# SamsungSAILMontreal/ghn3

Measured on AMD Instinct MI355X. Metric: predicted-params/sec (GHN fwd+bwd), ghn3xlm16, 256-node graphs, higher is better.
Workload: dtype f16; 1 GPU; ghn3xlm16 fwd+bwd, 1 synthetic 256-node graph(s) per GPU (seed 256000+), 86515016 predicted params per GPU, loss = sum of Frobenius norms of the predicted tensors; ghn_params=654365312, decoder_rows=1421, workspace_bytes=2436048640, zero_fill_bytes=2797339192, parallelism=dp1, index_mode=reference, loss=fused into the tile kernels

## Files before the change

### ghn3_amd/build.py

```python
import os
import subprocess
import sys
from concurrent.futures import ThreadPoolExecutor

HERE = os.path.dirname(os.path.abspath(__file__))
ROOT = os.path.dirname(HERE)
CSRC = os.path.join(HERE, 'csrc')
OUT_DIR = os.path.join(HERE, 'lib')
LIB = os.path.join(OUT_DIR, 'libghn3_hip.so')
SOURCES = ['gemm.hip', 'gemm_p8.hip', 'gemm_small.hip', 'gemm_x3.hip', 'gemm_x3d.hip', 'gemm_wg.hip', 'attention.hip', 'elementwise.hip', 'target_ops.hip', 'tnet_msa.hip', 'tnet_attn.hip', 'tnet_head.hip', 'tnet_wgrad.hip', 'tnet_join.hip', 'tnet_patch.hip', 'runtime.hip']
FLAGS = ['--offload-arch=gfx950', '-O3', '-std=c++17', '-fPIC', '-I' + os.path.join(ROOT, 'include'),
         '-I' + CSRC, '-Wno-unused-result'] + os.environ.get('GHN3_HIPCC_EXTRA', '').split()


def _hipcc():
    for cand in (os.environ.get('HIPCC'), '/opt/rocm/bin/hipcc', 'hipcc'):
        if cand and (os.path.isabs(cand) and os.path.exists(cand) or not os.path.isabs(cand)):
            return cand
    raise RuntimeError('hipcc not found')


def _stale(target, deps):
    if not os.path.exists(target):
        return True
    t = os.path.getmtime(target)
    return any(os.path.getmtime(d) > t for d in deps)


def source_hash():
    import hashlib
    h = hashlib.sha256()
    files = [os.path.join(CSRC, f) for f in sorted(os.listdir(CSRC)) if f.endswith(('.hip', '.h'))]
    files += [os.path.join(ROOT, 'include', 'ghn3_hip.h'), os.path.join(HERE, 'program.py')]
    for f in files:
        with open(f, 'rb') as fh:
            h.update(os.path.basename(f).encode() + b'\0' + fh.read())
    return h.hexdigest()[:16]


def build(force=False, verbose=True):
    os.makedirs(OUT_DIR, exist_ok=True)
    hipcc = _hipcc()
    headers = [os.path.join(ROOT, 'include', 'ghn3_hip.h'), os.path.join(CSRC, 'ghn3_internal.h'),
# ... 27 lines not shown
```

### ghn3_amd/csrc/ghn3_internal.h

```cpp
#pragma once
#include <hip/hip_runtime.h>
#include <stdint.h>
#include "ghn3_hip.h"

struct GemmProbDev {
    const float* A; const float* B; float* C;
    const float* bias; const float* residual; const float* aux_in; float* aux_out;
    const int* a_gather; const int* b_gather; const int* c_gather;
    int M, N, K, lda, ldb, ldc;
    int a_q, a_s, b_q, b_s, c_q, c_s;
    int bias_q, bias_s, bias_stride;
    int act, dact, flags;
    float alpha;
    int tile_start;
    int tiles_m, tiles_n;
    int ksplit, k_chunk;
    int order;
    int kq, ks;
    const int* lim;
    int lim_kind;
    int xcd_cols;
    int pin;
    int pin_first, pin_count;
    int pin_end, pin_total;
    const float* alpha_amax;
    int ln_kind;
    float ln_eps;
    const float* ln_p[6];
    const void* B2;
    const int* mtab;
};


int ghn3_gemm_init();
int ghn3_gemm_launch(const GemmProbDev* d_probs, int n_probs, int total_tiles, int a_mode, int b_mode,
                     int tile, int ctype, hipStream_t stream);

int ghn3_gemm_h16d_launch(const GemmProbDev* d_probs, int n_probs, int total_tiles, int tile, int ctype, int grid_cap,
                          hipStream_t stream);
int ghn3_gemm_p8_init();
int ghn3_gemm_p8_launch(const GemmProbDev* d_probs, int n_probs, int total_tiles, int ctype, int grid_cap,
                        hipStream_t stream);
int ghn3_gemm_p8w_launch(const GemmProbDev* d_probs, int n_probs, int total_tiles, int ctype, int grid_cap,
                         hipStream_t stream);
int ghn3_gemm_p8d_launch(const GemmProbDev* d_probs, int n_probs, int total_tiles, int ctype, int grid_cap,
                         hipStream_t stream);
int ghn3_gemm_x3_init();
int ghn3_gemm_x3_tile(int code, int slice, int* bm, int* bn);
int ghn3_gemm_x3_launch(const GemmProbDev* d_probs, int n_probs, int total_tiles, int code, int slice,
                        hipStream_t stream);
int ghn3_gemm_x3s_init();
int ghn3_gemm_x3s_tile(int code, int K, int ln_kind, int* bm, int* bn);
int ghn3_gemm_x3s_launch(const GemmProbDev* d_probs, const GemmProbDev* h_probs, int n_probs, int total_tiles, int code, int K,
                         int ln_kind, hipStream_t stream);
int ghn3_gemm_wg_launch(const GemmProbDev* d_probs, int n_probs, int total_tiles, int grid_cap, int tile_edge, hipStream_t stream);
int ghn3_gemm_small_launch(const GemmProbDev* d_probs, int n_probs, int total_tiles, int a_mode, int b_mode, int with_ln,
                           hipStream_t stream);

int ghn3_attn_init();
int ghn3_attn_fwd(float* out, const float* qkv, const float* bias, float* P, const int* n_nodes,
                  int B, int N, int C, int H, hipStream_t s);
int ghn3_attn_bwd(float* dqkv, const float* dO, const float* qkv, const float* P, const float* O, float* amax_out,
                  float* dBias, const int* n_nodes, int B, int N, int C, int H, int general, hipStream_t s);

int ghn3_graph_prologue(const int64_t* A, int* deg_in, int* deg_out, int* dist0, int* pair,
                        int B, int N, int V, hipStream_t s);
int ghn3_embed_nodes(float* x, const int* node_type, const int* shape_idx, const int* n_nodes, const int* node_off,
                     const float* E_type, const float* E_ch, const float* E_sp, const float* E_in,
                     const float* E_out, const float* E_dist, const int* deg_in, const int* deg_out,
                     const int* dist0, int B, int N, int C, hipStream_t s);
int ghn3_embed_bwd(const float* dx, const int* node_type, const int* shape_idx, const int* n_nodes,
                   const int* node_off, float* dE_type, float* dE_ch, float* dE_sp, float* dE_in, float* dE_out,
                   float* dE_dist, const int* deg_in, const int* deg_out, const int* dist0,
                   int B, int N, int C, int n_type, int n_ch, int n_sp, hipStream_t s);
int ghn3_edge_hidden(float* hid, const float* Pfw, const float* Pbw, int V, int C, hipStream_t s);
int ghn3_edge_hidden_bwd(float* dPfw, float* dPbw, float* dhid, const float* hid, int V, int C, hipStream_t s);
int ghn3_bias_gather(float* bias, const float* T, const int* pair, int B, int N, int H, hipStream_t s);
int ghn3_bias_hist(float* dT, const float* dBias, const int* pair, int B, int N, int H, int V, void* scratch,
                   int have_amax, hipStream_t s);
int ghn3_rowset_colsum(float* out, const float* X, const void* sets, int n_sets, int O, int I, hipStream_t s);
int ghn3_layernorm_fwd(float* y, float* x, const float* g, const float* b, float* mean, float* rstd, const float* add,
                       int n_add, int64_t add_stride, int rows, int C, float eps, hipStream_t s);
int ghn3_layernorm_bwd(float* dx, float* dy, const float* x, const float* g, const float* mean,
                       const float* rstd, const float* res, const float* add, int n_add, int64_t add_stride, int rows,
                       int C, hipStream_t s);
int ghn3_ln_param_grad(float* dg, float* db, const float* dy, const float* x, const float* mean,
                       const float* rstd, int rows, int C, int accum, hipStream_t s);
int ghn3_ln_param_grad_batch(float* gbase, const float* abase, const int64_t* table, int n_items, int rows, int C,
// ... 69 lines not shown
```

### ghn3_amd/csrc/runtime.hip

```cpp

#include "ghn3_internal.h"
#include <cstdarg>
#include <cstdio>
#include <cstring>
#include <vector>
#include <algorithm>

static thread_local char g_err[512] = "";

void ghn3_set_error(const char* fmt, ...) {
    va_list ap;
    va_start(ap, fmt);
    vsnprintf(g_err, sizeof(g_err), fmt, ap);
    va_end(ap);
}

extern "C" const char* ghn3_last_error(void) { return g_err; }
extern "C" int ghn3_abi_version(void) { return GHN3_ABI_VERSION; }

#define HIPCHK(expr)                                                                  \
    do {                                                                              \
        hipError_t e_ = (expr);                                                       \
        if (e_ != hipSuccess) {                                                       \
            ghn3_set_error("%s failed: %s", #expr, hipGetErrorString(e_));            \
// ... 145 lines not shown
    return GHN3_OK;
}
extern "C" int ghn3_profile_read(ghn3_ctx* c, double* ms, int64_t* launches, int reset) {
    if (!c) return GHN3_E_NOCTX;
    for (int i = 0; i < GHN3_OP_KIND_COUNT; ++i) {
        if (ms) ms[i] = c->ms[i];
        if (launches) launches[i] = c->launches[i];
        if (reset) { c->ms[i] = 0; c->launches[i] = 0; }
    }
    return GHN3_OK;
}
extern "C" int ghn3_profile_read_tags(ghn3_ctx* c, double* ms256, int64_t* n256, int reset) {
    if (!c) return GHN3_E_NOCTX;
    int rc = drain_pool(c);
    if (rc) return rc;
    for (int i = 0; i < 256; ++i) {
        if (ms256) ms256[i] = c->tag_ms[i];
        if (n256) n256[i] = c->tag_n[i];
        if (reset) { c->tag_ms[i] = 0; c->tag_n[i] = 0; }
    }
    return GHN3_OK;
}

struct Resolver {
    void* const* bufs; int n_bufs; bool bad;
    template <typename T> T* get(const ghn3_ref& r) {
        if (r.buf < 0) return nullptr;
        if (r.buf >= n_bufs || bufs[r.buf] == nullptr) { bad = true; return nullptr; }
        return reinterpret_cast<T*>(reinterpret_cast<char*>(bufs[r.buf]) + r.off);
    }
};

static int pick_tile(const ghn3_gemm_problem& p, int forced, int64_t op_t64) {
    if (p.flags & GHN3_GEMM_X3) {
        if (forced == 44 || forced == 45 || p.ln_kind)
            return (forced == 45 ? 7000 : 6000) + 100 * (p.ln_kind & 3) + ((p.K / 64) % 100);
        return 4000 + 10 * (((forced >= 40 && forced <= 42) ? forced : 40) - 40) + p.x3_slice / 64;
    }
    if (p.ln_kind) return 32;
    if (p.flags & GHN3_GEMM_OP16) {
        if (forced == 16 || forced == 24 || forced == 20 || forced == 25 || forced == 29 || forced == 30) return forced;
        if (forced == 28) {
            const bool kmap_ok = p.b_kq == 0 || p.b_kq % 64 == 0 || 64 % p.b_kq == 0;
            return (p.ksplit <= 1 && p.M >= 160 && (p.N & 3) == 0 && kmap_ok && p.a_gather.buf < 0 && p.b_gather.buf < 0 &&
                    p.c_gather.buf < 0) ? 28 : 16;
        }
        const int64_t t256 = (int64_t)((p.M + 255) / 256) * ((p.N + 255) / 256) * (p.ksplit > 1 ? p.ksplit : 1);
        const double eff = ((double)p.M / (((p.M + 255) / 256) * 256.0)) * ((double)p.N / (((p.N + 255) / 256) * 256.0));
        return (t256 >= 200 && eff >= 0.8) ? 24 : 16;
    }
    if (forced == 48 || forced == 49) {
        const bool ok = p.a_mode == GHN3_MODE_COL && p.b_mode == GHN3_MODE_COL && p.ksplit <= 1 && (p.M & 3) == 0 &&
                        (p.N & 3) == 0 && (p.ldc & 3) == 0 && (p.C.off & 15) == 0 && (p.lda & 3) == 0 && (p.ldb & 3) == 0 &&
                        (p.A.off & 15) == 0 && (p.B.off & 15) == 0 && p.a_gather.buf < 0 &&
                        p.b_gather.buf < 0 && p.c_gather.buf < 0 && !p.a_q && !p.b_q && !p.c_q && !p.bias_q &&
                        p.act == GHN3_ACT_NONE && p.dact == GHN3_DACT_NONE && p.residual.buf < 0 && p.aux_out.buf < 0 &&
                        (p.bias.buf < 0 || (p.flags & GHN3_GEMM_BIASGRAD));
        return ok ? forced : 64;
    }
    if (forced == 32 || forced == 64 || forced == 128) return forced;
    const double flops = 2.0 * p.M * p.N * (double)p.K;
    if (p.ksplit <= 1 && op_t64 <= 640 && flops <= 4e9 && p.K <= 8192) return 32;
    const int64_t t128 = (int64_t)((p.M + 127) / 128) * ((p.N + 127) / 128) * (p.ksplit > 1 ? p.ksplit : 1);
    if (p.M >= 96 && p.N >= 96 && t128 >= 192) return 128;
    return 64;
}

static inline bool is16(int tl) { return tl == 16 || tl == 24 || tl == 20 || tl == 25 || tl == 28 || tl == 29 || tl == 30; }

extern "C" int ghn3_run(ghn3_ctx* c, const ghn3_op* ops, int n_ops, const ghn3_gemm_problem* problems, int n_problems,
                        void* const* bufs, int n_bufs, void* stream_) {
    if (!c) return GHN3_E_NOCTX;
    if (n_ops < 0 || (n_ops > 0 && !ops) || n_bufs < 0) { ghn3_set_error("ghn3_run: bad arguments"); return GHN3_E_ARG; }
    hipStream_t stream = (hipStream_t)stream_;
    Resolver R{bufs, n_bufs, false};

    std::vector<std::vector<Launch>> fresh_launches;
    const std::vector<std::vector<Launch>>* launches = &fresh_launches;
    size_t need = 0;
    for (int k = 0; k < n_ops; ++k)
        if (ops[k].kind == GHN3_OP_GEMM) need += (size_t)ops[k].i[1];
    GemmProbDev* hs = nullptr; GemmProbDev* ds = nullptr;
    static const bool use_cache = !(getenv("GHN3_RUN_CACHE") && atoi(getenv("GHN3_RUN_CACHE")) == 0);
    int hit = -1;
    if (need > 0) {
        int rc = ctx_reserve(c, need);
        if (rc) return rc;
        if (n_problems < 0 || (n_problems > 0 && !problems)) { ghn3_set_error("ghn3_run: bad problem table"); return GHN3_E_ARG; }
        for (int i = 0; use_cache && i < kStageSlots && hit < 0; ++i) {
            const SlotCache& e = c->cache[i];
            if (e.valid && e.n_ops == n_ops && e.n_problems == n_problems && e.n_bufs == n_bufs &&
                memcmp(e.bufs.data(), bufs, (size_t)n_bufs * sizeof(void*)) == 0 &&
                memcmp(e.ops.data(), ops, (size_t)n_ops * sizeof(ghn3_op)) == 0 &&
                memcmp(e.problems.data(), problems, (size_t)n_problems * sizeof(ghn3_gemm_problem)) == 0)
                hit = i;
        }
    }
    if (hit >= 0) {
        SlotCache& e = c->cache[hit];
        e.stamp = ++c->clock;
        c->cache_hits++;
        hs = c->h_stage[hit]; ds = c->d_stage[hit];
        launches = &e.launches;
        if (e.up_stream != stream && c->ev_used[hit]) HIPCHK(hipStreamWaitEvent(stream, c->ev[hit], 0));
    } else if (need > 0) {
        int slot = 0;
        for (int i = 1; i < kStageSlots; ++i)
            if (c->cache[i].stamp < c->cache[slot].stamp) slot = i;
        c->cache[slot].valid = false;
        c->cache_misses++;
        if (c->ev_used[slot]) { HIPCHK(hipEventSynchronize(c->ev[slot])); c->ev_used[slot] = false; }
        hs = c->h_stage[slot]; ds = c->d_stage[slot];
        std::vector<std::vector<Launch>>& op_launches = fresh_launches;
        op_launches.resize(n_ops);
        size_t pos = 0;
        for (int k = 0; k < n_ops; ++k) {
            if (ops[k].kind != GHN3_OP_GEMM) continue;
            const int first = (int)ops[k].i[0], cnt = (int)ops[k].i[1], forced = (int)ops[k].i[2];
            if (first < 0 || cnt < 0 || first + cnt > n_problems) {
                ghn3_set_error("op %d: GEMM problem range [%d,%d) outside table of %d", k, first, first + cnt, n_problems);
                return GHN3_E_ARG;
            }
            int64_t op_t64 = 0;
            for (int q = first; q < first + cnt; ++q)
                op_t64 += (int64_t)((problems[q].M + 63) / 64) * ((problems[q].N + 63) / 64);
            std::vector<int> codes;
            for (int q = first; q < first + cnt; ++q) {
                if (problems[q].M <= 0 || problems[q].N <= 0) continue;
                const int tc = pick_tile(problems[q], forced, op_t64);
                if (std::find(codes.begin(), codes.end(), tc) == codes.end()) codes.push_back(tc);
            }
            std::sort(codes.begin(), codes.end());
            for (int am = 0; am < 2; ++am)
                for (int bm = 0; bm < 2; ++bm)
                    for (int tl : codes) {
                        Launch L{am, bm, tl, (int)pos, 0, 0, 0, 0};
                        int te = tl == 16 ? 128 : (tl == 24 || tl == 20 || tl == 25 || tl == 28 || tl == 29 || tl == 30) ? 256 : tl == 48 ? 64 : tl == 49 ? 128 : tl;
                        int te_n = (tl == 20 || tl == 30) ? 128 : te;
                        const bool x3 = tl >= 4000;
                        const bool x3old = x3 && tl < 5000;
                        if (x3old && !ghn3_gemm_x3_tile(40 + (tl - 4000) / 10, 64 * (tl % 10), &te, &te_n)) {
                            ghn3_set_error("op %d: no split-bf16 kernel for tile bucket %d (tile code %d, K slice %d)", k, tl,
                                           40 + (tl - 4000) / 10, 64 * (tl % 10));
                            return GHN3_E_LIMIT;
                        }
                        const int x3s_code = tl >= 7000 ? 45 : 44, x3s_ln = (tl / 100) % 10, x3s_k = 64 * (tl % 100);
                        if (tl >= 6000 && !ghn3_gemm_x3s_tile(x3s_code, x3s_k, x3s_ln, &te, &te_n)) {
                            ghn3_set_error("op %d: no staged split-bf16 kernel for tile code %d, K = %d, ln_kind %d "
                                           "(gemm_x3d.hip: K = C <= 384 with a prologue; 16 x 32 tiles also K = 3C / 4C)", k,
                                           x3s_code, x3s_k, x3s_ln);
                            return GHN3_E_LIMIT;
                        }
                        std::vector<int> members, pinned_m;
                        for (int q = first; q < first + cnt; ++q) {
                            const ghn3_gemm_problem& p = problems[q];
                            if (p.M <= 0 || p.N <= 0) continue;
                            if (p.a_mode != am || p.b_mode != bm || pick_tile(p, forced, op_t64) != tl) continue;
                            members.push_back(q);
                        }
                        const bool pin_ok = (tl == 16 || tl == 20 || tl == 28) && members.size() >= 8;
                        if (pin_ok) {
                            for (int x = 0; x < 8; ++x)
                                for (int q : members)
                                    if (problems[q].xcd_pin == x + 1 && problems[q].ksplit <= 1) pinned_m.push_back(q);
                            if (!pinned_m.empty()) {
                                std::vector<int> rest;
                                for (int q : members)
                                    if (!(problems[q].xcd_pin >= 1 && problems[q].xcd_pin <= 8 && problems[q].ksplit <= 1))
                                        rest.push_back(q);
                                members = pinned_m;
                                members.insert(members.end(), rest.begin(), rest.end());
                            }
                        }
                        const int n_pinned = (int)pinned_m.size();
                        int pin_local[8] = {0, 0, 0, 0, 0, 0, 0, 0}, pin_first[8] = {0, 0, 0, 0, 0, 0, 0, 0},
                            pin_count[8] = {0, 0, 0, 0, 0, 0, 0, 0};
                        int pin_end = 0;
                        if (n_pinned) {
                            for (int q : pinned_m) {
                                const ghn3_gemm_problem& p = problems[q];
                                const int tm_ = (tl == 28 && p.mtiles.buf >= 0) ? p.n_mtiles : (p.M + te - 1) / te;
                                pin_local[p.xcd_pin - 1] += tm_ * ((p.N + te_n - 1) / te_n);
                            }
                            for (int x = 0; x < 8; ++x) pin_end = std::max(pin_end, 8 * pin_local[x]);
                            for (int x = 0; x < 8; ++x) pin_local[x] = 0;
                            L.tiles = pin_end;
                        }
                        int member_k = 0;
                        for (int q : members) {
                            const ghn3_gemm_problem& p = problems[q];
                            const int member_i = member_k++;
                            const int pin_x = member_i < n_pinned ? p.xcd_pin - 1 : -1;
// ... 105 lines not shown
                            if (p.ln_kind) L.with_ln = 1;
                            for (int e = 0; e < 6; ++e) g.ln_p[e] = p.ln_kind ? R.get<const float>(p.ln_p[e]) : nullptr;
                            if (p.ln_kind) {
                                const bool ok = (p.ln_kind == 1 || p.ln_kind == 2) && p.a_mode == GHN3_MODE_ROW &&
                                                p.a_gather.buf < 0 && p.a_q == 0 && p.K <= 4096 && (p.K & 3) == 0 &&
                                                !(p.flags & GHN3_GEMM_OP16) && g.ln_p[0] &&
                                                (p.ln_kind == 1 ? g.ln_p[1] != nullptr
                                                                : (g.ln_p[1] && g.ln_p[2] && g.ln_p[3]));
                                if (!ok) {
                                    ghn3_set_error("op %d problem %d: the LayerNorm row prologue needs a ROW-mode fp32 A "
                                                   "without gather, K %% 4 == 0, K <= 4096 and its parameter refs", k, q);
                                    return GHN3_E_ARG;
                                }
                            }
                            g.order = (int64_t)p.M > (int64_t)p.N ? 1 : 0;
                            if (tl == 28) g.order = 0;
                            g.ksplit = p.ksplit > 1 ? p.ksplit : 1;
                            g.k_chunk = x3old ? p.x3_slice : x3 ? p.K : ((p.K + g.ksplit - 1) / g.ksplit + 63) / 64 * 64;
                            if (g.ksplit > 1 && (p.bias.buf >= 0 || p.act || p.dact || p.residual.buf >= 0 ||
                                                 p.aux_out.buf >= 0)) {
                                ghn3_set_error("op %d problem %d: split-K allows no epilogue but alpha", k, q);
                                return GHN3_E_ARG;
                            }
                            g.xcd_cols = 0;
                            if (pin_x >= 0) {
                            } else if (tl == 25 || tl == 29 || tl == 30) {
                                static const int64_t b_budget = getenv("GHN3_XCD_B_BYTES") ? atoll(getenv("GHN3_XCD_B_BYTES"))
                                                                                          : (int64_t)(5 << 19);
                                int G = 1;
                                while (G < 8 && (int64_t)p.N * p.K * 2 / G > b_budget && g.tiles_n >= 2 * G) G *= 2;
                                g.xcd_cols = G;
                                const int npg = (g.tiles_n + G - 1) / G, mpc = (g.tiles_m + 8 / G - 1) / (8 / G);
                                L.tiles += 8 * npg * mpc;
                            } else if (tl == 32 || tl == 48 || tl == 49 || x3) {
                                L.tiles += g.tiles_m * g.tiles_n;
                            } else {
                                const int per_split = g.order ? ((g.tiles_m + 7) / 8 * 8) * g.tiles_n
                                                              : g.tiles_m * ((g.tiles_n + 7) / 8 * 8);
                                L.tiles += per_split * g.ksplit;
                            }
                            L.count++;
                        }
                        if (n_pinned)
                            for (int x = 0; x < 8; ++x) {
                                hs[L.first + x].pin_first = pin_first[x];
                                hs[L.first + x].pin_count = pin_count[x];
                            }
                        if (L.count > 0) op_launches[k].push_back(L);
                    }
        }
        if (R.bad) { ghn3_set_error("ghn3_run: a GEMM problem references an absent buffer"); return GHN3_E_ARG; }
        HIPCHK(hipMemcpyAsync(ds, hs, pos * sizeof(GemmProbDev), hipMemcpyHostToDevice, stream));
        HIPCHK(hipEventRecord(c->ev[slot], stream));
        c->ev_used[slot] = true;
        if (use_cache) {
            SlotCache& e = c->cache[slot];
            e.n_ops = n_ops; e.n_problems = n_problems; e.n_bufs = n_bufs;
            e.ops.assign(ops, ops + n_ops);
            e.problems.assign(problems, problems + n_problems);
            e.bufs.assign(bufs, bufs + n_bufs);
            e.launches.swap(fresh_launches);
            launches = &e.launches;
            e.up_stream = stream;
            e.stamp = ++c->clock;
            e.valid = true;
        } else {
            c->cache[slot].stamp = ++c->clock;
// ... 44 lines not shown
                HIPCHK(hipEventRecord(c->ev_fork, main_stream));
                HIPCHK(hipStreamWaitEvent(c->side, c->ev_fork, 0));
                main_dirty = false;
            }
            side_dirty = true;
        } else {
            main_dirty = true;
        }
        hipStream_t stream = on_side ? c->side : main_stream;
        const bool timed = (c->profile == 2 || c->profile == 3) && (o.flags & GHN3_OPFLAG_TIMED);
        if (c->profile == 1) HIPCHK(hipEventRecord(c->pe0, stream));
        if (timed) {
            if (c->pool_used >= 8192) { int rc2 = drain_pool(c); if (rc2) return rc2; }
            if (c->pool->size() < 2 * (c->pool_used + 1)) {
                hipEvent_t e0, e1;
                HIPCHK(hipEventCreate(&e0));
                HIPCHK(hipEventCreate(&e1));
                c->pool->push_back(e0); c->pool->push_back(e1);
                c->pool_tag->push_back(0);
            }
            (*c->pool_tag)[c->pool_used] = (o.flags >> 16) & 255;
            HIPCHK(hipEventRecord((*c->pool)[2 * c->pool_used], stream));
        }
        switch (o.kind) {
        case GHN3_OP_NOP: break;
        case GHN3_OP_GEMM:
            for (const Launch& L : (*launches)[k]) {
                if (L.tile >= 6000)
                    rc = ghn3_gemm_x3s_launch(ds + L.first, hs + L.first, L.count, L.tiles, L.tile >= 7000 ? 45 : 44, L.max_slice,
                                              (L.tile / 100) % 10, stream);
                else if (L.tile >= 4000)
                    rc = ghn3_gemm_x3_launch(ds + L.first, L.count, L.tiles, 40 + (L.tile - 4000) / 10,
                                             64 * (L.tile % 10), stream);
                else if (L.tile == 48 || L.tile == 49)
                    rc = ghn3_gemm_wg_launch(ds + L.first, L.count, L.tiles, gemm_cap, L.tile == 49 ? 128 : 64, stream);
                else if (L.tile == 32)
                    rc = ghn3_gemm_small_launch(ds + L.first, L.count, L.tiles, L.a_mode, L.b_mode, L.with_ln, stream);
                else if (L.tile == 30)
                    rc = ghn3_gemm_p8d_launch(ds + L.first, L.count, L.tiles,
                                              (o.flags & 0xff) ? ((o.flags & 0xff) - 1) : c->ctype, gemm_cap, stream);
                else if (L.tile == 29)
                    rc = ghn3_gemm_p8w_launch(ds + L.first, L.count, L.tiles,
                                              (o.flags & 0xff) ? ((o.flags & 0xff) - 1) : c->ctype, gemm_cap, stream);
                else if (L.tile == 28)
                    rc = ghn3_gemm_p8_launch(ds + L.first, L.count, L.tiles,
                                             (o.flags & 0xff) ? ((o.flags & 0xff) - 1) : c->ctype, gemm_cap, stream);
                else if (is16(L.tile))
                    rc = ghn3_gemm_h16d_launch(ds + L.first, L.count, L.tiles,
                                               L.tile == 16 ? 128 : L.tile == 20 ? 20 : L.tile == 25 ? 25 : 256,
                                               (o.flags & 0xff) ? ((o.flags & 0xff) - 1) : c->ctype, gemm_cap,
                                               stream);
                else
                    rc = ghn3_gemm_launch(ds + L.first, L.count, L.tiles, L.a_mode, L.b_mode, L.tile,
                                          (o.flags & 0xff) ? ((o.flags & 0xff) - 1) : c->ctype, stream);
                if (rc) break;
            }
            break;
        case GHN3_OP_GRAPH_PROLOGUE:
            rc = ghn3_graph_prologue(R.get<const int64_t>(o.r[0]), R.get<int>(o.r[1]), R.get<int>(o.r[2]),
                                     R.get<int>(o.r[3]), R.get<int>(o.r[4]), (int)o.i[0], (int)o.i[1], (int)o.i[2],
                                     stream);
            break;
        case GHN3_OP_EMBED_NODES:
            rc = ghn3_embed_nodes(R.get<float>(o.r[0]), R.get<const int>(o.r[1]), R.get<const int>(o.r[2]),
                                  R.get<const int>(o.r[3]), R.get<const int>(o.r[4]), R.get<const float>(o.r[5]),
                                  R.get<const float>(o.r[6]), R.get<const float>(o.r[7]), R.get<const float>(o.r[8]),
// ... 253 lines not shown
```

### ghn3_amd/program.py

```python

import math
import os

import numpy as np

from . import _lib as L
from . import bookkeeping as bk

ALIGN = 256


def global_param_names():
    return ['ln.weight', 'ln.bias', 'embed.weight', 'shape_enc.embed_spatial.weight',
            'shape_enc.embed_channel.weight', 'gnn.0.centrality_embed_in.weight',
            'gnn.0.centrality_embed_out.weight', 'gnn.0.input_dist_embed.weight',
            'gnn.0.attn.edge_embed.embed.weight', 'gnn.0.attn.proj_e.0.weight', 'gnn.0.attn.proj_e.0.bias',
            'gnn.0.attn.proj_e.2.weight', 'gnn.0.attn.proj_e.2.bias',
            'decoder.fc.0.weight', 'decoder.fc.0.bias', 'decoder.conv.0.weight', 'decoder.conv.0.bias',
            'decoder.conv.2.weight', 'decoder.conv.2.bias', 'decoder.class_layer_predictor.1.weight',
            'decoder.class_layer_predictor.1.bias', 'decoder_1d.fc.0.weight', 'decoder_1d.fc.0.bias',
            'decoder_1d.fc.2.weight', 'decoder_1d.fc.2.bias', 'bias_class.1.weight', 'bias_class.1.bias']


LAYER_PARAM_NAMES = ['ln1.weight', 'ln1.bias', 'attn.to_qkv.weight', 'attn.to_out.0.weight', 'attn.to_out.0.bias',
# ... 4 lines not shown
def param_names(layers, layernorm=True):
    names = global_param_names()
    if not layernorm:
        names = [n for n in names if not n.startswith('ln.')]
    for l in range(layers):
        names += ['gnn.%d.%s' % (l, n) for n in LAYER_PARAM_NAMES]
    return names


def round_up(x, m):
    return (x + m - 1) // m * m


class Program:

    X_WS, X_IDX, X_EDGES, X_OUT, X_DOUT, X_TOK, X_SCAL, X_GRADFLAT, X_SHADOW, X_NORMG, X_COUNT = range(11)

    def __init__(self, cfg, node_infos, n_nodes, node_types, max_edge, nets, index_mode='reference',
                 training=True, predict_class_layers=True, reduce_graph=False, layernorm=True, weight_norm=True,
                 decoder_ctype=None, decoder_bwd_ctype=None, direct16=True, side_stream=True, graphormer_x3=None):
        self.cfg = cfg
        self.SIDE = L.OPFLAG_SIDE if side_stream else 0
        self.split_k2 = os.environ.get('GHN3_SPLIT_K2', '1') != '0'
        self.split_k2_min = int(os.environ.get('GHN3_SPLIT_K2_MIN', '768'))
        self.decoder_ctype = decoder_ctype
        if decoder_bwd_ctype is None:
            decoder_bwd_ctype = decoder_ctype
        self.decoder_bwd_ctype = decoder_bwd_ctype
        self.bwd_scaled = decoder_bwd_ctype == L.CT_F16
        self.direct16 = bool(direct16) and decoder_ctype in (L.CT_F16, L.CT_BF16) and (8 * int(cfg['hid'])) % 64 == 0
        self.d12_fwd_ctype = {'f32': L.CT_F32, 'f16': None}[os.environ.get('GHN3_D12_FWD', 'f32')]
        self.use_p8 = os.environ.get('GHN3_P8', '1') != '0'
        self.d1_bwd_ctype = {'f32': L.CT_F32, 'f16': None}[os.environ.get('GHN3_D1_BWD', 'f32')]
        self.C = C = int(cfg['hid'])
        if graphormer_x3 is None:
            graphormer_x3 = decoder_ctype in (L.CT_F16, L.CT_BF16) and os.environ.get('GHN3_X3', '1') != '0'
        self.x3 = bool(graphormer_x3) and C % 64 == 0 and 64 <= C <= 384
        self.x3s = self.x3 and C in (64, 128, 256, 384) and os.environ.get('GHN3_X3S', '1') != '0'
        self.x3f16 = self.x3s and os.environ.get('GHN3_X3_F16', '1') != '0'
        self.H = int(cfg['heads'])
        self.Lyr = int(cfg['layers'])
        self.K = int(cfg['num_classes'])
        self.max_shape = tuple(int(v) for v in cfg['max_shape'])
        self.S = self.max_shape[2]
        assert self.max_shape[2] == self.max_shape[3]
        self.layernorm = layernorm
        self.weight_norm = weight_norm
        self.training = training
        self.index_mode = index_mode
        self.names = param_names(self.Lyr, layernorm)
        self.P = len(self.names)
        self.slot = {n: i for i, n in enumerate(self.names)}
        self.B = len(n_nodes)
        self.n_nodes = [int(v) for v in n_nodes]
        self.N = max(self.n_nodes)
        self.V = int(max_edge) + 1
        if self.V + 1 > 257:
            raise ValueError('shortest-path length %d exceeds the 257-row edge embedding (graphormer.py:95-96)'
                             % max_edge)
        if self.N > 4096:
            raise ValueError('graphs with more than 4096 nodes are not supported (got %d)' % self.N)
        self._ops, self._probs, self._ln = [], [], {}
        self.tag_flops = {}
        self._ws = 0
        self._ws_names = {}
        self._idx_chunks, self._idx_size = [], 0
# ... 294 lines not shown

    _PROBLEM_REFS = ('A', 'B', 'C', 'bias', 'residual', 'aux_in', 'aux_out', 'a_gather', 'b_gather', 'c_gather', 'lim',
                     'alpha_amax', 'B2', 'mtiles')
    _PROBLEM_INTS = ('M', 'N', 'K', 'lda', 'ldb', 'ldc', 'a_mode', 'b_mode', 'a_q', 'a_s', 'b_q', 'b_s', 'c_q', 'c_s',
                     'bias_q', 'bias_s', 'bias_stride', 'act', 'dact', 'flags', 'b_kq', 'b_ks', 'x3_slice')

    def _pack_problems(self):
        n = len(self._probs)
        arr = np.zeros(n, dtype=L.PROBLEM_DT)
        if n == 0:
            return arr
        cols = list(zip(*self._probs))
        nr = len(self._PROBLEM_REFS)
        for k, name in enumerate(self._PROBLEM_REFS):
            ref = np.asarray(cols[k], dtype=np.int64).reshape(n, 2)
            arr[name]['buf'], arr[name]['off'] = ref[:, 0], ref[:, 1]
        for k, name in enumerate(self._PROBLEM_INTS):
            arr[name] = np.asarray(cols[nr + k], dtype=np.int64)
        k = nr + len(self._PROBLEM_INTS)
        arr['alpha'], arr['ksplit'], arr['lim_kind'], arr['xcd_pin'] = cols[k], cols[k + 1], cols[k + 2], cols[k + 3]
        arr['n_mtiles'] = cols[k + 4]
        arr['ln_p']['buf'] = -1
        for q, (kind, refs, eps) in self._ln.items():
            arr['ln_kind'][q], arr['ln_eps'][q] = kind, eps
            for e, ref in enumerate(refs):
                if ref is not None:
                    arr['ln_p']['buf'][q, e], arr['ln_p']['off'][q, e] = ref
        return arr

    TAG_D3_FWD, TAG_D3_DGRAD, TAG_D3_WGRAD, TAG_D2_FWD, TAG_D1_FWD, TAG_TILE_FWD, TAG_TILE_BWD, TAG_D2_BWD, \
        TAG_D1_BWD = range(1, 10)
    TAG_NAMES = {1: 'w2_fwd', 2: 'w2_dgrad', 3: 'w2_wgrad', 4: 'w0_fwd', 5: 'fc_fwd', 6: 'tile_fwd', 7: 'tile_bwd',
                 8: 'w0_bwd', 9: 'fc_bwd'}

    def gemm_op(self, first, count=None, tile=0, ctype=None, tag=0, side=False, flops=None, grid_cap=0):
        if count is None:
            count = len(self._probs) - first
        if count > 0:
            if tag and ctype is None:
                ctype = self.decoder_ctype
            flags = 0 if ctype is None else 1 + ctype
            if side:
                flags |= self.SIDE
            if tag:
                flags |= L.OPFLAG_TIMED | (tag << 16)
                fl = flops if flops is not None else \
                    sum(2.0 * int(p[14]) * int(p[15]) * int(p[16]) for p in self._probs[first:first + count])
                self.tag_flops[tag] = self.tag_flops.get(tag, 0.0) + fl
            self.op(L.OP_GEMM, ints=(first, count, tile, grid_cap), flags=flags)

    @staticmethod
    def _row_parts(rows):
        main = rows // 128 * 128
        rem = rows - main
        if main >= 128 and 0 < rem <= 64:
            return [(0, main), (main, rem)]
        return [(0, rows)]

    P8_COST = {3: 1.72, 4: 2.0, 5: 2.42}
    P8_MI = tuple(int(v) for v in os.environ.get('GHN3_P8_MI', '3,4,5').split(','))

    @classmethod
    def row_tiles(cls, ext):
        ext = np.asarray(ext, dtype=np.int64)
        R = len(ext)
        if cls.P8_FINE:
# ... 511 lines not shown
            p0 = self.gemm(xe, self.pref(W1), h1d, self.n1, 2 * C, C, C, C, 2 * C, bias=self.pref(b1),
                           act=L.ACT_RELU, a_gather=r_src1)
            self.gemm_op(p0)
            p0 = len(self._probs)
            if self.n1_plain:
                self.gemm(h1d, self.pref(W2d), w1d, self.n1_plain, 2 * mc, 2 * C, 2 * C, 2 * C, 2 * mc,
                          bias=self.pref(b2d))
            if self.n1_clsb:
                self.gemm(self.wref('h1d', self.n1_plain * 2 * C), self.pref(W2d),
                          self.wref('w1d', self.n1_plain * 2 * mc), self.n1_clsb, 2 * mc, 2 * C, 2 * C, 2 * C, 2 * mc,
                          bias=self.pref(b2d), act=L.ACT_RELU)
            self.gemm_op(p0)
            if self.n1_clsb:
                cbout = self.wsf('cbout', self.n1_clsb * ldK)
                p0 = self.gemm(self.wref('w1d', self.n1_plain * 2 * mc + mc), self.pref(Wb), cbout, self.n1_clsb, K,
                               mc, 2 * mc, mc, ldK, bias=self.pref(bb))
                self.gemm_op(p0)

        if self.SIDE:
            self.op(L.OP_JOIN)
        if M > 0:
            t = self.wsf('t', M * 4 * C)
            u = self.wsf('u', M * 8 * C)
            self.d1 = []
            p0 = len(self._probs)
            for p in np.unique(self.row_pos):
                rws = np.nonzero(self.row_pos == p)[0].astype(np.int32)
                r_rows = self.idx(rws)
                r_src = self.idx(self.row_src[rws])
                self.d1.append((int(p), len(rws), r_rows, r_src))
                self.gemm(xe, self.pref(Wfc, int(p) * C), t, len(rws), 4 * C, C, C, S2 * C, 4 * C,
                          bias=self.pref(bfc, int(p)), bias_stride=S2, act=L.ACT_RELU, a_gather=r_src,
                          c_gather=r_rows)
            self.gemm_op(p0, tag=self.TAG_D1_FWD, ctype=self.d12_fwd_ctype)
            d2_fix = self.decoder_ctype in (L.CT_F16, L.CT_BF16) and os.environ.get('GHN3_D2_FIX', '1') != '0' and \
                self.d12_fwd_ctype == L.CT_F32
            p0 = self.gemm(t, self.pref(W0), u, M, 8 * C, 4 * C, 4 * C, 4 * C, 8 * C, bias=self.pref(b0),
                           act=L.ACT_NONE if d2_fix else L.ACT_RELU)
            self.gemm_op(p0, tag=self.TAG_D2_FWD, ctype=self.decoder_ctype if d2_fix else self.d12_fwd_ctype)
            if d2_fix:
                self.op(L.OP_RELU_FIX, refs=(u, t, self.pref(W0), self.pref(b0)),
                        ints=(M, 8 * C, 8 * C, 4 * C, 0, 0),
                        floats=(float(os.environ.get('GHN3_RELU_FIX_TAU', '5e-3')),))
            p0 = len(self._probs)
            tiles_floats = 0
            for gg in self.gemm_groups:
                gg['tile_off'] = tiles_floats
                for g in gg['members']:
                    g['tile_off'] = tiles_floats + (g['row0'] - gg['row0']) * gg['ld']
                tiles_floats += round_up(gg['rows'] * gg['ld'], 64)
            for g in self.conv_groups:
                if 'resize' in g:
                    g['rs_off'] = tiles_floats
                    tiles_floats += round_up(g['resize'][0] * g['resize'][1] * g['ld'], 64)
            self.tiles_floats = tiles_floats
            tiles = self.wsf('tiles', tiles_floats)
            use16 = any(g['op16'] for g in self.gemm_groups)
            if use16:
                fct = self.decoder_ctype
                self.op(L.OP_JOIN)
                self.uh = self.ws16('uh', M * 8 * C)
                self.cast16((self.xbuf(self.X_WS), 0),
                            [dict(src_off=u[1] // 4, rows=M, cols=8 * C, ld_src=8 * C, straight=(self.uh, 8 * C, fct))])
            fl = 0.0
            for g in self.gemm_groups:
                fl += sum(2.0 * sb['rows'] * sb['cols'] * 8 * C for sb in g['subs'])
                if g['op16'] and g['p8'] and self.P8_BALANCED:
# ... 817 lines not shown
                d2_tile = int(os.environ.get('GHN3_D2_DGRAD_TILE', '0'))
                ks = int(os.environ.get('GHN3_D2_DGRAD_KS', '0')) or \
                    max(1, min(4, 320 // max(1, ((M + 127) // 128) * ((4 * C + 127) // 128))))
                while ks > 1 and (8 * C) % (64 * ks):
                    ks -= 1
                if ks > 1:
                    kc = 8 * C // ks
                    planes = self.wsf('d_t_parts', (ks - 1) * M * 4 * C)
                    p0 = len(self._probs)
                    for j in range(ks):
                        dst = d_t if j == 0 else (planes[0], planes[1] + 4 * (j - 1) * M * 4 * C)
                        self.gemm(self.href(duh + j * kc), self.sref(self.w0hT + j * kc), dst, M, 4 * C, kc, 8 * C, 8 * C,
                                  4 * C, op16=True, alpha_amax=amax_u)
                    self.gemm_op(p0, ctype=bct, tag=self.TAG_D2_BWD, flops=2.0 * M * 4 * C * 8 * C, tile=d2_tile)
                    self.op(L.OP_DACT, refs=(d_t, t, self.NONE, planes),
                            ints=(M, 4 * C, 4 * C, L.DACT_RELU, ks - 1, M * 4 * C, M))
                else:
                    p0 = self.gemm(self.href(duh), self.sref(self.w0hT), d_t, M, 4 * C, 8 * C, 8 * C, 8 * C, 4 * C,
                                   dact=L.DACT_RELU, aux_in=t, op16=True, alpha_amax=amax_u)
                    self.gemm_op(p0, ctype=bct, tag=self.TAG_D2_BWD)
            else:
                p0 = self.gemm(d_u, t, self.gref(W0), 8 * C, 4 * C, M, 8 * C, 4 * C, 4 * C, a_mode=L.MODE_COL,
                               b_mode=L.MODE_COL, accum=True, dbias=self.gref(b0))
                self.gemm_op(p0, tag=self.TAG_D2_BWD, side=True)
                p0 = self.gemm(d_u, self.pref(W0), d_t, M, 4 * C, 8 * C, 8 * C, 4 * C, 4 * C, a_mode=L.MODE_ROW,
                               b_mode=L.MODE_COL, dact=L.DACT_RELU, aux_in=t)
                self.gemm_op(p0, tag=self.TAG_D2_BWD)
            p0 = len(self._probs)
            for (p, cnt, r_rows, r_src) in self.d1:
                self.gemm(d_t, self.pref(Wfc, p * C), d_rows, cnt, C, 4 * C, 4 * C, S2 * C, C, a_mode=L.MODE_ROW,
                          b_mode=L.MODE_COL, a_gather=r_rows, c_gather=r_rows)
            self.gemm_op(p0, tag=self.TAG_D1_BWD, ctype=self.d1_bwd_ctype, tile=int(os.environ.get('GHN3_D1_DGRAD_TILE', '0')))
            p0 = len(self._probs)
            for (p, cnt, r_rows, r_src) in self.d1:
                self.gemm(d_t, xe, self.gref(Wfc, p * C), 4 * C, C, cnt, 4 * C, C, S2 * C, a_mode=L.MODE_COL,
                          b_mode=L.MODE_COL, a_gather=r_rows, b_gather=r_src, accum=True,
                          dbias=self.gref(bfc, p), dbias_stride=S2)
            self.gemm_op(p0, tag=self.TAG_D1_BWD, side=True, ctype=self.d1_bwd_ctype)
        if not early_1d:
            decoder_1d_bwd(False)
        self.bwd_split = len(self._ops)
        all_src = np.concatenate([self.row_src, self.oned_src]) if (M + n1) else np.zeros(0, dtype=np.int32)
        order = np.argsort(all_src, kind='stable').astype(np.int32)
        counts = np.bincount(all_src, minlength=rows)[:rows]
        seg_ptr = np.concatenate([[0], np.cumsum(counts)]).astype(np.int32)
        d_xe = self.wsf('d_xe', rows * C)
        if early_1d:
            self.op(L.OP_JOIN, ints=(2, 0))
        self.op(L.OP_ROWSEG_SUM, refs=(d_xe, d_rows, self.idx(seg_ptr), self.idx(order)), ints=(rows, C, C, C, 0))

        dxa = self.wsf('dxa', rows * C)
        do = self.wsf('do', rows * C)
        nb_ = round_up(4 * B * H * N * N, 16)
        dBias = self.wsf('dBias', nb_ // 4 + 2 * V * V * H + 16)
        hist = (dBias[0], dBias[1] + nb_)
        hist_amax = (dBias[0], dBias[1] + nb_ + 8 * V * V * H)
        self.op(L.OP_MEMSET0, refs=(dBias,), ints=(nb_ + 8 * V * V * H + 16,))
        xL = self.wref('x%d' % self.Lyr)
        if self.layernorm:
            self.op(L.OP_LAYERNORM_BWD, refs=(dxa, d_xe, xL, self.pref('ln.weight'), self.wref('mf'), self.wref('rf'),
                                              self.NONE), ints=(rows, C))
            self.op(L.OP_LN_PARAM_GRAD, refs=(self.gref('ln.weight'), self.gref('ln.bias'), d_xe, xL,
                                              self.wref('mf'), self.wref('rf')), ints=(rows, C, 1), flags=self.SIDE)
            g_cur = dxa
        else:
            g_cur = d_xe
        bias = self.wref('bias')
        pending_ln1 = None
        side_group = max(1, int(os.environ.get('GHN3_SIDE_GROUP', '4'))) if self.SIDE else 1
        side_pending = []
        layer_side = []
# ... 119 lines not shown
```

Measured before the change: 15.39 billion predicted-params/s.

## Add streaming FC kernels for decoder-1 forward and weight-gradient GEMMs

Adds a dedicated fp32 MFMA kernel family for the decoder's per-position FC layers. The forward kernel keeps a 64-column weight slab in registers and streams the gathered input rows through LDS. The wgrad kernel covers a 64-row slab of the output and streams over K, writing the result directly instead of accumulating. The goal is to replace generic tiled GEMMs on these skinny, many-small-problem shapes and to avoid re-reading the weights. This relies on the weight-gradient output being written once, not accumulated, and on the bias gradient being accumulated non-atomically, which could be wrong if problems overlap.

```diff
diff --git a/ghn3_amd/build.py b/ghn3_amd/build.py
--- a/ghn3_amd/build.py
+++ b/ghn3_amd/build.py
@@ -8,7 +8,7 @@
 CSRC = os.path.join(HERE, 'csrc')
 OUT_DIR = os.path.join(HERE, 'lib')
 LIB = os.path.join(OUT_DIR, 'libghn3_hip.so')
-SOURCES = ['gemm.hip', 'gemm_p8.hip', 'gemm_small.hip', 'gemm_x3.hip', 'gemm_x3d.hip', 'gemm_wg.hip', 'attention.hip', 'elementwise.hip', 'target_ops.hip', 'tnet_msa.hip', 'tnet_attn.hip', 'tnet_head.hip', 'tnet_wgrad.hip', 'tnet_join.hip', 'tnet_patch.hip', 'runtime.hip']
+SOURCES = ['gemm.hip', 'gemm_p8.hip', 'gemm_small.hip', 'gemm_x3.hip', 'gemm_x3d.hip', 'gemm_wg.hip', 'gemm_fc.hip', 'attention.hip', 'elementwise.hip', 'target_ops.hip', 'tnet_msa.hip', 'tnet_attn.hip', 'tnet_head.hip', 'tnet_wgrad.hip', 'tnet_join.hip', 'tnet_patch.hip', 'runtime.hip']
 FLAGS = ['--offload-arch=gfx950', '-O3', '-std=c++17', '-fPIC', '-I' + os.path.join(ROOT, 'include'),
          '-I' + CSRC, '-Wno-unused-result'] + os.environ.get('GHN3_HIPCC_EXTRA', '').split()
 
diff --git a/ghn3_amd/csrc/gemm_fc.hip b/ghn3_amd/csrc/gemm_fc.hip
--- /dev/null
+++ b/ghn3_amd/csrc/gemm_fc.hip
@@ -0,0 +1,234 @@
+
+#include "ghn3_internal.h"
+
+#define GAS __attribute__((address_space(1)))
+typedef float f32x4 __attribute__((ext_vector_type(4)));
+typedef f32x4 GAS* gf4;
+typedef const f32x4 GAS* gcf4;
+typedef const int GAS* gci;
+
+namespace {
+
+constexpr int FC_SLAB = 64;
+
+__device__ __forceinline__ const GemmProbDev* fc_find(const GemmProbDev* probs, int n_probs, int tile) {
+    int lo = 0, hi = n_probs - 1;
+    while (lo < hi) {
+        const int mid = (lo + hi + 1) >> 1;
+        if (probs[mid].tile_start <= tile) lo = mid; else hi = mid - 1;
+    }
+    return probs + lo;
+}
+
+template <int K>
+__global__ __launch_bounds__(256) void fc_fwd_kernel(const GemmProbDev* __restrict__ probs, int n_probs) {
+    constexpr int LDX = K + 4;
+    constexpr int F4 = K / 4;
+    constexpr int NL = (4 * F4 + 63) / 64;
+    __shared__ __attribute__((aligned(16))) float xs[16 * LDX];
+    const GemmProbDev* P = fc_find(probs, n_probs, blockIdx.x);
+    const int tid = threadIdx.x, lane = tid & 63, wave = tid >> 6, c = lane & 15, g = lane >> 4;
+    const int M = P->M, N = P->N, lda = P->lda;
+    const int n0 = (blockIdx.x - P->tile_start) * FC_SLAB + wave * 16;
+    const bool live = n0 < N;
+    const float GAS* Ag = (const float GAS*)P->A;
+    gci ag = (gci)P->a_gather;
+    gci cg = (gci)P->c_gather;
+    const f32x4 zero = f32x4{0.f, 0.f, 0.f, 0.f};
+
+    f32x4 w[K / 16];
+    {
+        f32x4 st[4][NL];
+        const float GAS* Bg = (const float GAS*)P->B + (int64_t)n0 * P->ldb;
+#pragma unroll
+        for (int t = 0; t < 4; ++t)
+#pragma unroll
+            for (int e = 0; e < NL; ++e) {
+                const int i = 64 * e + lane, r = i / F4;
+                st[t][e] = (live && i < 4 * F4) ? *reinterpret_cast<gcf4>(Bg + (int64_t)(4 * t + r) * P->ldb + 4 * (i - r * F4)) : zero;
+            }
+        float* ws = xs + wave * 4 * LDX;
+#pragma unroll
+        for (int t = 0; t < 4; ++t) {
+            if (t) __syncthreads();
+#pragma unroll
+            for (int e = 0; e < NL; ++e) {
+                const int i = 64 * e + lane, r = i / F4;
+                if (i < 4 * F4) *reinterpret_cast<f32x4*>(ws + r * LDX + 4 * (i - r * F4)) = st[t][e];
+            }
+            __syncthreads();
+            if ((c >> 2) == t) {
+#pragma unroll
+                for (int q = 0; q < K / 16; ++q) w[q] = *reinterpret_cast<const f32x4*>(ws + (c & 3) * LDX + 16 * q + 4 * g);
+            }
+        }
+    }
+    f32x4 bv = zero;
+    if (live && P->bias) {
+        const float GAS* b = (const float GAS*)P->bias;
+#pragma unroll
+        for (int r = 0; r < 4; ++r) bv[r] = b[(int64_t)(n0 + 4 * g + r) * P->bias_stride];
+    }
+    const float alpha = P->alpha;
+    const bool relu = P->act == GHN3_ACT_RELU;
+    float GAS* C = (float GAS*)P->C;
+
+    for (int m0 = 0; m0 < M; m0 += 16) {
+        __syncthreads();
+        for (int i = tid; i < 16 * F4; i += 256) {
+            const int r = i / F4, f = i - r * F4;
+            const int m = m0 + r;
+            f32x4 v = zero;
+            if (m < M) v = *reinterpret_cast<gcf4>(Ag + (int64_t)(ag ? ag[m] : m) * lda + 4 * f);
+            *reinterpret_cast<f32x4*>(xs + r * LDX + 4 * f) = v;
+        }
+        __syncthreads();
+        if (!live) continue;
+        f32x4 acc0 = zero, acc1 = zero;
+        const float* xr = xs + c * LDX + 4 * g;
+#pragma unroll
+        for (int q = 0; q < K / 16; ++q) {
+            const f32x4 x = *reinterpret_cast<const f32x4*>(xr + 16 * q);
+            acc0 = __builtin_amdgcn_mfma_f32_16x16x4f32(w[q][0], x[0], acc0, 0, 0, 0);
+            acc1 = __builtin_amdgcn_mfma_f32_16x16x4f32(w[q][1], x[1], acc1, 0, 0, 0);
+            acc0 = __builtin_amdgcn_mfma_f32_16x16x4f32(w[q][2], x[2], acc0, 0, 0, 0);
+            acc1 = __builtin_amdgcn_mfma_f32_16x16x4f32(w[q][3], x[3], acc1, 0, 0, 0);
+        }
+        const int m = m0 + c;
+        if (m < M) {
+            f32x4 v;
+#pragma unroll
+            for (int r = 0; r < 4; ++r) {
+                v[r] = (acc0[r] + acc1[r]) * alpha + bv[r];
+                if (relu) v[r] = fmaxf(v[r], 0.f);
+            }
+            *reinterpret_cast<gf4>(C + (int64_t)(cg ? cg[m] : m) * P->ldc + n0 + 4 * g) = v;
+        }
+    }
+}
+
+template <int NC>
+__global__ __launch_bounds__(256) void fc_wgrad_kernel(const GemmProbDev* __restrict__ probs, int n_probs) {
+    constexpr int KC = 16;
+    constexpr int LDB = NC + 16, LDA = FC_SLAB + 16;
+    constexpr int F4 = NC / 4, NT = NC / 16;
+    __shared__ __attribute__((aligned(16))) float xs[KC * LDB];
+    __shared__ __attribute__((aligned(16))) float ds[KC * LDA];
+    const GemmProbDev* P = fc_find(probs, n_probs, blockIdx.x);
+    const int tid = threadIdx.x, lane = tid & 63, wave = tid >> 6, c = lane & 15, g = lane >> 4;
+    const int M = P->M, K = P->K, lda = P->lda, ldb = P->ldb;
+    const int m0 = (blockIdx.x - P->tile_start) * FC_SLAB;
+    const float GAS* Ag = (const float GAS*)P->A;
+    const float GAS* Bg = (const float GAS*)P->B;
+    gci ag = (gci)P->a_gather;
+    gci bg = (gci)P->b_gather;
+    const f32x4 zero = f32x4{0.f, 0.f, 0.f, 0.f};
+
+    f32x4 acc[NT];
+#pragma unroll
+    for (int j = 0; j < NT; ++j) acc[j] = zero;
+    float bsum = 0.f;
+
+    for (int k0 = 0; k0 < K; k0 += KC) {
+        if (k0) __syncthreads();
+        for (int i = tid; i < KC * F4; i += 256) {
+            const int r = i / F4, f = i - r * F4;
+            const int k = k0 + r;
+            f32x4 v = zero;
+            if (k < K) v = *reinterpret_cast<gcf4>(Bg + (int64_t)(bg ? bg[k] : k) * ldb + 4 * f);
+            *reinterpret_cast<f32x4*>(xs + r * LDB + 4 * f) = v;
+        }
+        {
+            const int r = tid >> 4, f = tid & 15;
+            const int k = k0 + r, m = m0 + 4 * f;
+            f32x4 v = zero;
+            if (k < K && m < M) v = *reinterpret_cast<gcf4>(Ag + (int64_t)(ag ? ag[k] : k) * lda + m);
+            *reinterpret_cast<f32x4*>(ds + r * LDA + 4 * f) = v;
+        }
+        __syncthreads();
+#pragma unroll
+        for (int s = 0; s < KC / 4; ++s) {
+            if (k0 + 4 * s >= K) break;
+            const int kk = 4 * s + g;
+            const float d = ds[kk * LDA + wave * 16 + c];
+            bsum += d;
+            const float* xr = xs + kk * LDB + c;
+#pragma unroll
+            for (int j = 0; j < NT; ++j) acc[j] = __builtin_amdgcn_mfma_f32_16x16x4f32(xr[16 * j], d, acc[j], 0, 0, 0);
+        }
+    }
+
+    const float alpha = P->alpha;
+    float* ws = xs + wave * 4 * LDB;
+    float GAS* Cg = (float GAS*)P->C;
+#pragma unroll
+    for (int t = 0; t < 4; ++t) {
+        __syncthreads();
+        if ((c >> 2) == t) {
+#pragma unroll
+            for (int j = 0; j < NT; ++j) *reinterpret_cast<f32x4*>(ws + (c & 3) * LDB + 16 * j + 4 * g) = acc[j] * alpha;
+        }
+        __syncthreads();
+        for (int i = lane; i < 4 * F4; i += 64) {
+            const int r = i / F4, f = i - r * F4;
+            const int m = m0 + wave * 16 + 4 * t + r;
+            if (m < M) *reinterpret_cast<gf4>(Cg + (int64_t)m * P->ldc + 4 * f) = *reinterpret_cast<const f32x4*>(ws + r * LDB + 4 * f);
+        }
+    }
+    if (P->flags & GHN3_GEMM_BIASGRAD) {
+        bsum += __shfl_xor(bsum, 16, 64);
+        bsum += __shfl_xor(bsum, 32, 64);
+        const int m = m0 + wave * 16 + c;
+        if (g == 0 && m < M) {
+            float GAS* db = (float GAS*)P->bias + (int64_t)m * P->bias_stride;
+            *db += bsum;
+        }
+    }
+}
+
+template <int D>
+void fc_launch(int a_mode, const GemmProbDev* d_probs, int n_probs, int total_tiles, hipStream_t stream) {
+    if (a_mode == GHN3_MODE_ROW)
+        hipLaunchKernelGGL(fc_fwd_kernel<D>, dim3(total_tiles), dim3(256), 0, stream, d_probs, n_probs);
+    else
+        hipLaunchKernelGGL(fc_wgrad_kernel<D>, dim3(total_tiles), dim3(256), 0, stream, d_probs, n_probs);
+}
+
+}
+
+int ghn3_gemm_fc_dim(const ghn3_gemm_problem& p) {
+    if (p.flags & ~(unsigned)GHN3_GEMM_BIASGRAD) return 0;
+    if (p.ln_kind || p.ksplit > 1 || p.a_q || p.b_q || p.c_q || p.bias_q || p.residual.buf >= 0 || p.aux_in.buf >= 0 ||
+        p.aux_out.buf >= 0 || p.dact != GHN3_DACT_NONE || p.M < 1 || p.N < 1 || p.K < 1 || (p.ldc & 3) || (p.C.off & 15) ||
+        (p.lda & 3) || (p.ldb & 3) || (p.A.off & 15) || (p.B.off & 15))
+        return 0;
+    auto dim_ok = [](int d) { return d == 32 || d == 64 || d == 128 || d == 256 || d == 384; };
+    if (p.a_mode == GHN3_MODE_ROW && p.b_mode == GHN3_MODE_ROW) {
+        if ((p.flags & GHN3_GEMM_BIASGRAD) || p.b_gather.buf >= 0 || (p.N & 15) || !dim_ok(p.K) ||
+            (p.act != GHN3_ACT_NONE && p.act != GHN3_ACT_RELU))
+            return 0;
+        return p.K;
+    }
+    if (p.a_mode == GHN3_MODE_COL && p.b_mode == GHN3_MODE_COL) {
+        if (p.c_gather.buf >= 0 || (p.M & 3) || !dim_ok(p.N) || p.act != GHN3_ACT_NONE ||
+            (p.bias.buf >= 0 && !(p.flags & GHN3_GEMM_BIASGRAD)))
+            return 0;
+        return p.N;
+    }
+    return 0;
+}
+
+int ghn3_gemm_fc_launch(const GemmProbDev* d_probs, int n_probs, int total_tiles, int a_mode, int dim, hipStream_t stream) {
+    if (n_probs <= 0 || total_tiles <= 0) return GHN3_OK;
+    switch (dim) {
+    case 32: fc_launch<32>(a_mode, d_probs, n_probs, total_tiles, stream); break;
+    case 64: fc_launch<64>(a_mode, d_probs, n_probs, total_tiles, stream); break;
+    case 128: fc_launch<128>(a_mode, d_probs, n_probs, total_tiles, stream); break;
+    case 256: fc_launch<256>(a_mode, d_probs, n_probs, total_tiles, stream); break;
+    case 384: fc_launch<384>(a_mode, d_probs, n_probs, total_tiles, stream); break;
+    default: ghn3_set_error("fc gemm: no kernel for a streamed dimension of %d", dim); return GHN3_E_LIMIT;
+    }
+    hipError_t e = hipGetLastError();
+    if (e != hipSuccess) { ghn3_set_error("fc gemm launch: %s", hipGetErrorString(e)); return GHN3_E_HIP; }
+    return GHN3_OK;
+}
diff --git a/ghn3_amd/csrc/ghn3_internal.h b/ghn3_amd/csrc/ghn3_internal.h
--- a/ghn3_amd/csrc/ghn3_internal.h
+++ b/ghn3_amd/csrc/ghn3_internal.h
@@ -54,6 +54,8 @@
 int ghn3_gemm_x3s_launch(const GemmProbDev* d_probs, const GemmProbDev* h_probs, int n_probs, int total_tiles, int code, int K,
                          int ln_kind, hipStream_t stream);
 int ghn3_gemm_wg_launch(const GemmProbDev* d_probs, int n_probs, int total_tiles, int grid_cap, int tile_edge, hipStream_t stream);
+int ghn3_gemm_fc_dim(const ghn3_gemm_problem& p);
+int ghn3_gemm_fc_launch(const GemmProbDev* d_probs, int n_probs, int total_tiles, int a_mode, int dim, hipStream_t stream);
 int ghn3_gemm_small_launch(const GemmProbDev* d_probs, int n_probs, int total_tiles, int a_mode, int b_mode, int with_ln,
                            hipStream_t stream);
 
diff --git a/ghn3_amd/csrc/runtime.hip b/ghn3_amd/csrc/runtime.hip
--- a/ghn3_amd/csrc/runtime.hip
+++ b/ghn3_amd/csrc/runtime.hip
@@ -201,6 +201,11 @@
 };
 
 static int pick_tile(const ghn3_gemm_problem& p, int forced, int64_t op_t64) {
+    if (forced == 52) {
+        const int d = ghn3_gemm_fc_dim(p);
+        if (d) return 520 + d / 16;
+        forced = 0;
+    }
     if (p.flags & GHN3_GEMM_X3) {
         if (forced == 44 || forced == 45 || p.ln_kind)
             return (forced == 45 ? 7000 : 6000) + 100 * (p.ln_kind & 3) + ((p.K / 64) % 100);
@@ -235,6 +240,7 @@
     return 64;
 }
 
+static inline bool is_fc(int tl) { return tl >= 520 && tl < 560; }
 static inline bool is16(int tl) { return tl == 16 || tl == 24 || tl == 20 || tl == 25 || tl == 28 || tl == 29 || tl == 30; }
 
 extern "C" int ghn3_run(ghn3_ctx* c, const ghn3_op* ops, int n_ops, const ghn3_gemm_problem* problems, int n_problems,
@@ -285,7 +291,9 @@
         size_t pos = 0;
         for (int k = 0; k < n_ops; ++k) {
             if (ops[k].kind != GHN3_OP_GEMM) continue;
-            const int first = (int)ops[k].i[0], cnt = (int)ops[k].i[1], forced = (int)ops[k].i[2];
+            const int first = (int)ops[k].i[0], cnt = (int)ops[k].i[1];
+            int forced = (int)ops[k].i[2];
+            if (forced == 52 && (ops[k].flags & 0xff) != 1 + GHN3_CT_F32) forced = 0;
             if (first < 0 || cnt < 0 || first + cnt > n_problems) {
                 ghn3_set_error("op %d: GEMM problem range [%d,%d) outside table of %d", k, first, first + cnt, n_problems);
                 return GHN3_E_ARG;
@@ -307,6 +315,11 @@
                         int te = tl == 16 ? 128 : (tl == 24 || tl == 20 || tl == 25 || tl == 28 || tl == 29 || tl == 30) ? 256 : tl == 48 ? 64 : tl == 49 ? 128 : tl;
                         int te_n = (tl == 20 || tl == 30) ? 128 : te;
                         const bool x3 = tl >= 4000;
+                        const bool fc = is_fc(tl);
+                        if (fc) {
+                            te = am == GHN3_MODE_ROW ? (1 << 24) : 64;
+                            te_n = am == GHN3_MODE_ROW ? 64 : (1 << 24);
+                        }
                         const bool x3old = x3 && tl < 5000;
                         if (x3old && !ghn3_gemm_x3_tile(40 + (tl - 4000) / 10, 64 * (tl % 10), &te, &te_n)) {
                             ghn3_set_error("op %d: no split-bf16 kernel for tile bucket %d (tile code %d, K slice %d)", k, tl,
@@ -327,6 +340,12 @@
                             if (p.a_mode != am || p.b_mode != bm || pick_tile(p, forced, op_t64) != tl) continue;
                             members.push_back(q);
                         }
+                        if (fc)
+                            std::stable_sort(members.begin(), members.end(), [&](int x, int y) {
+                                const int rx = am == GHN3_MODE_ROW ? problems[x].M : problems[x].K;
+                                const int ry = am == GHN3_MODE_ROW ? problems[y].M : problems[y].K;
+                                return rx > ry;
+                            });
                         const bool pin_ok = (tl == 16 || tl == 20 || tl == 28) && members.size() >= 8;
                         if (pin_ok) {
                             for (int x = 0; x < 8; ++x)
@@ -498,7 +517,7 @@
                                 g.xcd_cols = G;
                                 const int npg = (g.tiles_n + G - 1) / G, mpc = (g.tiles_m + 8 / G - 1) / (8 / G);
                                 L.tiles += 8 * npg * mpc;
-                            } else if (tl == 32 || tl == 48 || tl == 49 || x3) {
+                            } else if (tl == 32 || tl == 48 || tl == 49 || x3 || fc) {
                                 L.tiles += g.tiles_m * g.tiles_n;
                             } else {
                                 const int per_split = g.order ? ((g.tiles_m + 7) / 8 * 8) * g.tiles_n
@@ -609,6 +628,8 @@
                 else if (L.tile >= 4000)
                     rc = ghn3_gemm_x3_launch(ds + L.first, L.count, L.tiles, 40 + (L.tile - 4000) / 10,
                                              64 * (L.tile % 10), stream);
+                else if (is_fc(L.tile))
+                    rc = ghn3_gemm_fc_launch(ds + L.first, L.count, L.tiles, L.a_mode, (L.tile - 520) * 16, stream);
                 else if (L.tile == 48 || L.tile == 49)
                     rc = ghn3_gemm_wg_launch(ds + L.first, L.count, L.tiles, gemm_cap, L.tile == 49 ? 128 : 64, stream);
                 else if (L.tile == 32)
diff --git a/ghn3_amd/program.py b/ghn3_amd/program.py
--- a/ghn3_amd/program.py
+++ b/ghn3_amd/program.py
@@ -60,6 +60,7 @@
         self.d12_fwd_ctype = {'f32': L.CT_F32, 'f16': None}[os.environ.get('GHN3_D12_FWD', 'f32')]
         self.use_p8 = os.environ.get('GHN3_P8', '1') != '0'
         self.d1_bwd_ctype = {'f32': L.CT_F32, 'f16': None}[os.environ.get('GHN3_D1_BWD', 'f32')]
+        self.d1_stream = os.environ.get('GHN3_D1_STREAM', '1') != '0'
         self.C = C = int(cfg['hid'])
         if graphormer_x3 is None:
             graphormer_x3 = decoder_ctype in (L.CT_F16, L.CT_BF16) and os.environ.get('GHN3_X3', '1') != '0'
@@ -420,6 +421,9 @@
         TAG_D1_BWD = range(1, 10)
     TAG_NAMES = {1: 'w2_fwd', 2: 'w2_dgrad', 3: 'w2_wgrad', 4: 'w0_fwd', 5: 'fc_fwd', 6: 'tile_fwd', 7: 'tile_bwd',
                  8: 'w0_bwd', 9: 'fc_bwd'}
+
+    def d1_tile(self, ctype):
+        return 52 if self.d1_stream and ctype == L.CT_F32 and self.C in (32, 64, 128, 256, 384) else 0
 
     def gemm_op(self, first, count=None, tile=0, ctype=None, tag=0, side=False, flops=None, grid_cap=0):
         if count is None:
@@ -997,7 +1001,7 @@
                 self.gemm(xe, self.pref(Wfc, int(p) * C), t, len(rws), 4 * C, C, C, S2 * C, 4 * C,
                           bias=self.pref(bfc, int(p)), bias_stride=S2, act=L.ACT_RELU, a_gather=r_src,
                           c_gather=r_rows)
-            self.gemm_op(p0, tag=self.TAG_D1_FWD, ctype=self.d12_fwd_ctype)
+            self.gemm_op(p0, tag=self.TAG_D1_FWD, ctype=self.d12_fwd_ctype, tile=self.d1_tile(self.d12_fwd_ctype))
             d2_fix = self.decoder_ctype in (L.CT_F16, L.CT_BF16) and os.environ.get('GHN3_D2_FIX', '1') != '0' and \
                 self.d12_fwd_ctype == L.CT_F32
             p0 = self.gemm(t, self.pref(W0), u, M, 8 * C, 4 * C, 4 * C, 4 * C, 8 * C, bias=self.pref(b0),
@@ -1881,11 +1885,12 @@
                           b_mode=L.MODE_COL, a_gather=r_rows, c_gather=r_rows)
             self.gemm_op(p0, tag=self.TAG_D1_BWD, ctype=self.d1_bwd_ctype, tile=int(os.environ.get('GHN3_D1_DGRAD_TILE', '0')))
             p0 = len(self._probs)
+            wg_tile = self.d1_tile(self.d1_bwd_ctype)
             for (p, cnt, r_rows, r_src) in self.d1:
                 self.gemm(d_t, xe, self.gref(Wfc, p * C), 4 * C, C, cnt, 4 * C, C, S2 * C, a_mode=L.MODE_COL,
-                          b_mode=L.MODE_COL, a_gather=r_rows, b_gather=r_src, accum=True,
+                          b_mode=L.MODE_COL, a_gather=r_rows, b_gather=r_src, accum=not wg_tile,
                           dbias=self.gref(bfc, p), dbias_stride=S2)
-            self.gemm_op(p0, tag=self.TAG_D1_BWD, side=True, ctype=self.d1_bwd_ctype)
+            self.gemm_op(p0, tag=self.TAG_D1_BWD, side=True, ctype=self.d1_bwd_ctype, tile=wg_tile)
         if not early_1d:
             decoder_1d_bwd(False)
         self.bwd_split = len(self._ops)
```

Result: no change. 15.42 billion predicted-params/s (median of 6 runs) (+0.2%).
